# wildltr/ptranking

Hardware: AMD Instinct MI355X
Metric: queries/sec fwd+bwd LambdaRank, MSLR-WEB30K-shaped list_len=128 (higher is better)
Workload: dtype f32

## Files before the change

ptranking_amd/csrc/scorer_x6.hip:

```cpp
#include "ptr_mlp.h"

namespace ptr {

constexpr int kX6Pieces = kX6SliceBytes / 1024;
constexpr int kX6Ring = 6;

__host__ __device__ inline size_t x6_lds_bytes(int NL) { return (size_t)kX6Ring * kX6SliceBytes + ((size_t)NL * kHP + kHP + 16) * sizeof(float); }

__device__ __forceinline__ float relu1(float x) { return __builtin_amdgcn_fmed3f(x, 0.0f, 3.0e38f); }

__global__ void __launch_bounds__(256) x6_prep_kernel(const float *__restrict__ P, int F, int NL, uint8_t *__restrict__ img) {
    const int idx = blockIdx.x * 256 + threadIdx.x;
    const int n1 = x6_n1(F), ns = x6_nslices(F, NL);
    if (idx >= ns * kX6Rows * 4) return;
    const int g = idx & 3, row = (idx >> 2) % kX6Rows, sl = idx / (4 * kX6Rows);
    const int layer = sl < n1 ? 0 : 1 + (sl - n1) / 4, s = sl < n1 ? sl : (sl - n1) % 4;
    const int K = layer == 0 ? F : kH;
    const float *W = P + off_W(layer, F);
    Frag f[3];
#pragma unroll
    for (int h = 0; h < 2; ++h) {
        f32x4 v;
#pragma unroll
        for (int c = 0; c < 4; ++c) {
            const int k = layer == 0 ? 32 * s + 8 * g + 4 * h + c : 32 * s + 16 * h + 4 * g + c;
            v[c] = (row < kH && k < K) ? W[(size_t)row * K + k] : 0.0f;
            if (layer > 0 && row < kH && k == kH) v[c] = P[off_b(layer, F) + row];
        }
        split_pack4(v, f, 2 * h);
    }
#pragma unroll
    for (int p = 0; p < 3; ++p)
        *reinterpret_cast<u32x4 *>(img + (size_t)sl * kX6SliceBytes + (size_t)p * kX6PlaneBytes + (size_t)(row >> 4) * 1024 + g * 256 + (row & 15) * 16) = f[p].q;
}

using x6_rsrc = __amdgpu_buffer_rsrc_t;
__device__ __forceinline__ x6_rsrc x6_srd(void *p, uint32_t bytes) { return __builtin_amdgcn_make_buffer_rsrc(p, 0, (int)bytes, 0x00020000); }
__device__ __forceinline__ void x6_store16(x6_rsrc srd, uint32_t off, f32x4 v) {
    __builtin_amdgcn_raw_buffer_store_b128(__builtin_bit_cast(u32x4, v), srd, (int)off, 0, 0);
}
__device__ __forceinline__ f32x4 x6_load16(x6_rsrc srd, uint32_t voff, uint32_t soff) {
    return __builtin_bit_cast(f32x4, __builtin_amdgcn_raw_buffer_load_b128(srd, (int)voff, (int)soff, 0));
}
__device__ __forceinline__ void x6_store4(x6_rsrc srd, uint32_t off, float v) { __builtin_amdgcn_raw_buffer_store_b32(__builtin_bit_cast(uint32_t, v), srd, (int)off, 0, 0); }
constexpr uint32_t kX6Oob = 0xFFFFC000u;
constexpr uint64_t kX6BufLimit = 0xFFFFC000ull;

#define X6_MFMA(A, B, C) __builtin_amdgcn_mfma_f32_16x16x32_bf16((A).v, (B).v, (C), 0, 0, 0)

#define X6_SB() __builtin_amdgcn_sched_barrier(0)
#define X6_TSTRIDE 1024
#define X6_MIX(NM, NV)                                                                                     \
    do {                                                                                                   \
        _Pragma("unroll") for (int i_ = 0; i_ < (NM); ++i_) {                                              \
            __builtin_amdgcn_sched_group_barrier(0x008, 1, 0);                                             \
            __builtin_amdgcn_sched_group_barrier(0x002, (NV), 0);                                          \
        }                                                                                                  \
    } while (0)
template <int... Ks> struct X6K {};
template <int R, int K0, int... Ks> constexpr int x6_kget(X6K<K0, Ks...>) { if constexpr (R == 0) return K0; else return x6_kget<R - 1>(X6K<Ks...>{}); }

template <bool TRAIN, bool STORE, int DT>
__global__ void __launch_bounds__(16 / DT * 64, DT == 4 ? 1 : 2)
mlp_fwd_x6_kernel(const float *__restrict__ X, const float *__restrict__ P, const uint8_t *__restrict__ img, MlpArgs a,
                  float *__restrict__ preds, float *__restrict__ acts) {
    extern __shared__ __attribute__((aligned(16))) uint8_t smem_x6[];
    constexpr int NW = 16 / DT, RPT = 16 * DT, PW = (kX6Pieces + NW - 1) / NW;
    const int F = a.F, NL = a.NL, R = a.R;
    float *Bs = reinterpret_cast<float *>(smem_x6 + (size_t)kX6Ring * kX6SliceBytes);
    float *Wo = Bs + (size_t)NL * kHP;
    const int tid = threadIdx.x;
    for (int i = tid; i < NL * kHP; i += NW * 64) { const int l = i / kHP, c = i - l * kHP; Bs[i] = c < kH ? P[off_b(l, F) + c] : 0.0f; }
    for (int i = tid; i < kHP + 16; i += NW * 64) Wo[i] = i < kH ? P[off_wout(NL, F) + i] : (i == kHP ? P[off_wout(NL, F) + kH] : 0.0f);
    __syncthreads();
    const float b_out = Wo[kHP];

    const int lane = tid & 63, j = lane & 15, g = lane >> 4, wave = __builtin_amdgcn_readfirstlane(tid >> 6);
    const int ntiles = (R + RPT - 1) / RPT;
    const uint32_t thr = drop_thr(a.p_drop);
    const float scale = TRAIN ? 1.0f / (1.0f - a.p_drop) : 1.0f;
    const int n1 = x6_n1(F), ns = n1 + 4 * (NL - 1);
    const uint32_t ring = lds_byte_addr(smem_x6);
    const uint32_t lane_a = ring + (uint32_t)(lane * 16);

    int dma_slice = 0, dma_slot = 0;
    auto dma_issue = [&]() __attribute__((always_inline)) {
        const uint8_t *src = img + (size_t)dma_slice * kX6SliceBytes + lane * 16;
        const uint32_t dst = ring + (uint32_t)dma_slot * kX6SliceBytes;
#pragma unroll
        for (int i = 0; i < PW; ++i) {
            int q = wave * PW + i;
            q = q < kX6Pieces ? q : kX6Pieces - 1;
            glds16(src + q * 1024, __builtin_amdgcn_readfirstlane(dst + (uint32_t)q * 1024));
        }
        dma_slice = dma_slice + 1 == ns ? 0 : dma_slice + 1;
        dma_slot = dma_slot + 1 == kX6Ring ? 0 : dma_slot + 1;
    };
#pragma unroll 1
    for (int d = 0; d < kX6Ring - 1; ++d) dma_issue();
    static_assert(kX6Ring == 6 && (PW == 3 || PW == 6), "the vmcnt immediates below are PW * (kX6Ring - 2) and PW * (kX6Ring - 3) (+ the store margin)");
    if constexpr (STORE && DT == 2) {
#pragma unroll
        for (int i = 0; i < 6; ++i)
            glds16(img + (size_t)i * 1024 + lane * 16, __builtin_amdgcn_readfirstlane(ring + (uint32_t)(kX6Ring - 1) * kX6SliceBytes + (uint32_t)i * 1024));
    }
    if constexpr (DT == 4) asm volatile("s_waitcnt vmcnt(24)\n\ts_barrier" ::: "memory");
    else if constexpr (STORE) asm volatile("s_waitcnt vmcnt(18)\n\ts_barrier" ::: "memory");
    else asm volatile("s_waitcnt vmcnt(12)\n\ts_barrier" ::: "memory");
    int cur_slot = 0;
#ifdef PTR_X6_TRACE
    unsigned long long *trace = reinterpret_cast<unsigned long long *>(const_cast<uint8_t *>(img) + (size_t)ns * kX6SliceBytes) + wave * 256;
    int nstamp = 0;
#define X6_STAMP() do { if (blockIdx.x == 0 && lane == 0 && nstamp < 254) { trace[nstamp++] = clock64(); trace[nstamp & 1 ? 255 : 254] = wall_clock64(); if (nstamp == 1) trace[253] = wall_clock64(); } } while (0)
#else
#define X6_STAMP() do { } while (0)
#endif
    auto slice_sync = [&]() __attribute__((always_inline)) -> uint32_t {
        X6_STAMP();
        if constexpr (DT == 4) { if constexpr (STORE) asm volatile("s_waitcnt vmcnt(46)\n\ts_barrier" ::: "memory"); else asm volatile("s_waitcnt vmcnt(18)\n\ts_barrier" ::: "memory"); }
        else if constexpr (STORE) asm volatile("s_waitcnt vmcnt(23)\n\ts_barrier" ::: "memory");
        else asm volatile("s_waitcnt vmcnt(9)\n\ts_barrier" ::: "memory");
        X6_STAMP();
        dma_issue();
        cur_slot = cur_slot + 1 == kX6Ring ? 0 : cur_slot + 1;
        return lane_a + (uint32_t)cur_slot * kX6SliceBytes;
    };

    uint32_t bs_base = lds_byte_addr(Bs) + (uint32_t)g * 16;
    asm volatile("" : "+v"(bs_base));
    uint32_t wo_delta = (uint32_t)NL * (kHP * 4);
    asm volatile("" : "+s"(wo_delta));
    auto lds4 = [](uint32_t base, int byte_off) __attribute__((always_inline)) { return *reinterpret_cast<lds_f32x4 *>((uintptr_t)(base + (uint32_t)byte_off)); };
    const uint32_t nrt = (uint32_t)act_row_tiles(R), layer_bytes = nrt * (uint32_t)(kActTile * 4);
    const x6_rsrc xsrd = x6_srd(const_cast<float *>(X), (uint32_t)R * (uint32_t)(F * 4));
    const x6_rsrc psrd = x6_srd(preds, (uint32_t)R * 4u);
    const x6_rsrc asrd = x6_srd(acts, STORE ? (uint32_t)NL * layer_bytes : 0u);
    f32x4 acc[kMT][DT];
    Frag bp[4][DT][3];
    Frag bfx[2][DT][3];
    f32x4 raw[2][DT][2];
    Frag af[2][3];
    using I0 = std::integral_constant<int, 0>; using I1 = std::integral_constant<int, 1>;

    auto read_a = [&](Frag (&buf)[3], uint32_t abase, int mt) __attribute__((always_inline)) {
#pragma unroll
        for (int p = 0; p < 3; ++p) buf[p].q = *reinterpret_cast<lds_u32x4 *>((uintptr_t)(abase + (uint32_t)(p * kX6PlaneBytes + mt * 1024)));
    };
    auto mma_tile = [&](const Frag (&buf)[3], auto mt_, const Frag (&bf)[DT][3]) __attribute__((always_inline)) {
        constexpr int mt = decltype(mt_)::value;
#pragma unroll
        for (int q = 0; q < 6; ++q)
#pragma unroll
            for (int dt = 0; dt < DT; ++dt) acc[mt][dt] = X6_MFMA(buf[kSixA[q]], bf[dt][kSixB[q]], acc[mt][dt]);
    };
    auto mma_tile_tail = [&](const Frag (&buf)[3], auto mt_, const Frag (&bf)[DT][3]) __attribute__((always_inline)) {
        constexpr int mt = decltype(mt_)::value;
#pragma unroll
        for (int q = 0; q < 6; ++q)
#pragma unroll
            for (int dt = 0; dt < DT; ++dt)
                acc[mt][dt] = __builtin_amdgcn_mfma_f32_16x16x16bf16_1k(__builtin_bit_cast(i16x4, u32x2{buf[kSixA[q]].u[0], buf[kSixA[q]].u[1]}),
                                                                         __builtin_bit_cast(i16x4, u32x2{bf[dt][kSixB[q]].u[0], bf[dt][kSixB[q]].u[1]}), acc[mt][dt], 0, 0, 0);
    };
    auto slice_step = [&](auto ap_, uint32_t abase, const Frag (&bf)[DT][3], auto &&work, auto ks_, auto late_, auto tail_) __attribute__((always_inline)) -> uint32_t {
        constexpr int AP = decltype(ap_)::value;
        constexpr bool LATE = decltype(late_)::value;
        constexpr bool TAIL16 = decltype(tail_)::value;
        uint32_t nb = 0;
        static_for<kMT>([&](auto r_) __attribute__((always_inline)) {
            constexpr int r = decltype(r_)::value;
            constexpr int K = x6_kget<r>(decltype(ks_){});
            if constexpr (r == 3) nb = slice_sync();
            if constexpr (!LATE) {
                if constexpr (r < kMT - 1) read_a(af[AP ^ ((r + 1) & 1)], abase, r + 1);
                else read_a(af[AP ^ 1], nb, 0);
                X6_SB();
            }
            if constexpr (TAIL16) mma_tile_tail(af[AP ^ (r & 1)], r_, bf); else mma_tile(af[AP ^ (r & 1)], r_, bf);
            work(r_);
            if constexpr (K > 0) X6_MIX(6 * DT, K);
            X6_SB();
            if constexpr (LATE) {
                if constexpr (r < kMT - 1) read_a(af[AP ^ ((r + 1) & 1)], abase, r + 1);
                else read_a(af[AP ^ 1], nb, 0);
                X6_SB();
            }
        });
        return nb;
    };
    using Early = std::false_type;
    using Full = std::false_type;
    using Tail16 = std::true_type;
    using LateE = std::bool_constant<TRAIN>;
    using KNone = X6K<0, 0, 0, 0, 0, 0, 0>;
    auto nowork = [](auto) __attribute__((always_inline)) {};

    const int npass = (ntiles + NW * (int)gridDim.x - 1) / (NW * (int)gridDim.x);
    auto tile_of = [&](int it) __attribute__((always_inline)) { return (it * (int)gridDim.x + (int)blockIdx.x) * NW + wave; };
    uint32_t jX = (uint32_t)j * (uint32_t)(F * 4) + (uint32_t)g * 32, l16 = (uint32_t)(j * 64 + g * 16);
    uint32_t jH = (uint32_t)j * kDropRowMul + (uint32_t)g * kDropFgMul + a.seed_lo, jK = jH + (uint32_t)g * kDropFgMul;
    asm volatile("" : "+v"(jX), "+v"(l16), "+v"(jH), "+v"(jK));
    auto load_xq = [&](f32x4 (&rw)[DT][2], int t32, int s, int q) __attribute__((always_inline)) {
        const int dt = q >> 1, h = q & 1;
        const int left = F * 4 - 128 * s - 16 * h;
        const int ng = left <= 0 ? 0 : (left + 31) >> 5;
        const uint64_t cmask = ng >= 4 ? ~0ull : ((1ull << (16 * ng)) - 1ull);
        const uint64_t m = __builtin_amdgcn_ballot_w64(j < R - t32 - 16 * dt) & cmask;
        const uint32_t vo = __builtin_amdgcn_inverse_ballot_w64(m) ? jX : kX6Oob;
        const uint32_t so = (uint32_t)(t32 + 16 * dt) * (uint32_t)(F * 4);
        rw[dt][h] = x6_load16(xsrd, vo, so + (uint32_t)(128 * s + 16 * h));
    };
    auto make_bq = [&](const f32x4 (&rw)[DT][2], int t32, int s, Frag (&bf)[DT][3], int q) __attribute__((always_inline)) {
        const int dt = q >> 1, h = q & 1;
        f32x4 v = rw[dt][h];
        if constexpr (TRAIN) {
            uint32_t w0, w1;
            drop_bits_key(jK + ((uint32_t)(t32 + 16 * dt) * kDropRowMul + (uint32_t)(8 * s + h) * kDropFgMul), a.seed_hi, w0, w1);
            v = drop4(v, w0, w1, thr, scale);
        }
        split_pack4(v, bf[dt], 2 * h);
    };
    auto bias_init = [&]() __attribute__((always_inline)) {
#pragma unroll
        for (int mt = 0; mt < kMT; ++mt) {
            const f32x4 b4 = lds4(bs_base, 64 * mt);
            acc[mt][0] = b4; acc[mt][1] = b4;
        }
    };

    {
        const int t0 = tile_of(0) * RPT;
#pragma unroll
        for (int q = 0; q < 2 * DT; ++q) { load_xq(raw[0], t0, 0, q); load_xq(raw[1], t0, n1 > 1 ? 1 : 0, q); }
#pragma unroll
        for (int q = 0; q < 2 * DT; ++q) { make_bq(raw[0], t0, 0, bfx[0], q); load_xq(raw[0], t0, n1 > 2 ? 2 : 0, q); }
    }
    bias_init();
    uint32_t abase = lane_a;
    read_a(af[0], abase, 0);
    constexpr int KX = TRAIN ? 4 : 2, KE = TRAIN ? 9 : 5;

#pragma unroll 1
    for (int it = 0; it < npass; ++it) {
        const int tile = tile_of(it), tile_next = tile_of(it + 1);
        const int t32 = tile * RPT, t32n = tile_next * RPT;
        auto store_off = [&](int layer, int dt) __attribute__((always_inline)) {
            const uint32_t rt = (uint32_t)(t32 + 16 * dt) >> 4;
            uint32_t o = rt < nrt ? l16 + (rt * (uint32_t)(kActTile * 4) + (uint32_t)layer * layer_bytes) : kX6Oob;
            asm volatile("" : "+v"(o));
            return o;
        };
        auto epilogue = [&](auto mt_, int site) __attribute__((always_inline)) {
            constexpr int mt = decltype(mt_)::value;
#pragma unroll
            for (int dt = 0; dt < DT; ++dt) {
                f32x4 h = acc[mt][dt];
                acc[mt][dt] = f32x4{0.0f, 0.0f, 0.0f, 0.0f};
#pragma unroll
                for (int c = 0; c < 4; ++c) h[c] = relu1(h[c]);
                if constexpr (TRAIN) {
                    uint32_t w0, w1;
                    drop_bits_key(jH + ((uint32_t)(t32 + 16 * dt) * kDropRowMul + (uint32_t)(4 * mt) * kDropFgMul + (uint32_t)site * kDropSiteMul), a.seed_hi, w0, w1);
                    h = drop4(h, w0, w1, thr, scale);
                }
                if constexpr (STORE) {
                    f32x4 o = h;
                    if (mt == kMT - 1 && g == 1) o[0] = 1.0f;
                    x6_store16(asrd, store_off(site - 1, dt) + X6_TSTRIDE * mt, o);
                }
                split_pack4(h, bp[mt >> 1][dt], 2 * (mt & 1));
                if (mt == kMT - 1) {
                    bp[3][dt][0].u[0] |= g == 1 ? 0x3F80u : 0u;
                }
            }
        };
        float sc[DT];
#pragma unroll
        for (int dt = 0; dt < DT; ++dt) sc[dt] = 0.0f;
        auto epilogue_out = [&](auto mt_) __attribute__((always_inline)) {
            constexpr int mt = decltype(mt_)::value;
            const f32x4 w4 = lds4(bs_base + wo_delta, 64 * mt);
            const f32x4 bn = lds4(bs_base, 64 * mt);
#pragma unroll
            for (int dt = 0; dt < DT; ++dt) {
                f32x4 h = acc[mt][dt];
                acc[mt][dt] = bn;
#pragma unroll
                for (int c = 0; c < 4; ++c) { h[c] = relu1(h[c]); sc[dt] = fmaf(h[c], w4[c], sc[dt]); }
                if constexpr (STORE) x6_store16(asrd, store_off(NL - 1, dt) + X6_TSTRIDE * mt, h);
            }
        };

        auto l1_step = [&](auto par_, int s) __attribute__((always_inline)) {
            constexpr int PAR = decltype(par_)::value;
            abase = slice_step(par_, abase, bfx[PAR], [&](auto r_) __attribute__((always_inline)) {
                constexpr int r = decltype(r_)::value;
                auto quarter = [&](int q) __attribute__((always_inline)) { make_bq(raw[PAR ^ 1], t32, s + 1, bfx[PAR ^ 1], q); load_xq(raw[PAR ^ 1], t32, s + 3 < n1 ? s + 3 : 0, q); };
                if constexpr (DT == 2) {
                    constexpr int q = r == 0 ? 0 : r == 1 ? 1 : r == 3 ? 2 : r == 4 ? 3 : -1;
                    if constexpr (q >= 0) quarter(q);
                } else {
                    if constexpr (r == 0) { quarter(0); quarter(1); } else quarter(r + 1);
                }
            }, std::conditional_t<DT == 2, X6K<KX, KX, 0, KX, KX, 0, 0>, X6K<KX, KX / 2, KX / 2, KX / 2, KX / 2, KX / 2, KX / 2>>{}, Early{}, Full{});
        };
        auto l1_last = [&](auto par_) __attribute__((always_inline)) {
            constexpr int PAR = decltype(par_)::value;
            abase = slice_step(par_, abase, bfx[PAR], [&](auto r_) __attribute__((always_inline)) {
                constexpr int r = decltype(r_)::value;
                if constexpr (r > 0) epilogue(std::integral_constant<int, r - 1>{}, 1);
            }, X6K<0, KE, KE, KE, KE, KE, KE>{}, LateE{}, Full{});
            epilogue(std::integral_constant<int, kMT - 1>{}, 1);
            if constexpr (PAR == 0) {
#pragma unroll
                for (int p = 0; p < 3; ++p) af[0][p].q = af[1][p].q;
            }
        };
        int s = 0;
        for (; s + 2 <= n1 - 1; s += 2) { l1_step(I0{}, s); l1_step(I1{}, s + 1); }
        if (s < n1 - 1) { l1_step(I0{}, s); l1_last(I1{}); } else { l1_last(I0{}); }

        auto hidden = [&](auto lastlayer_, int l) __attribute__((always_inline)) {
            constexpr bool LAST = decltype(lastlayer_)::value;
            abase = slice_step(I0{}, abase, bp[0], nowork, KNone{}, Early{}, Full{});
            abase = slice_step(I1{}, abase, bp[1], nowork, KNone{}, Early{}, Full{});
            if constexpr (LAST) {
#pragma unroll
                for (int q = 0; q < 2 * DT; ++q) { load_xq(raw[0], t32n, 0, q); load_xq(raw[1], t32n, n1 > 1 ? 1 : 0, q); }
                X6_SB();
            }
            abase = slice_step(I0{}, abase, bp[2], nowork, KNone{}, Early{}, Full{});
            if constexpr (LAST) {
                abase = slice_step(I1{}, abase, bp[3], [&](auto r_) __attribute__((always_inline)) {
                    constexpr int r = decltype(r_)::value;
                    auto quarter = [&](int q) __attribute__((always_inline)) { make_bq(raw[0], t32n, 0, bfx[0], q); load_xq(raw[0], t32n, n1 > 2 ? 2 : 0, q); };
                    if constexpr (DT == 2) { if constexpr (r < 4) quarter(r); }
                    else if constexpr (r < 4) { quarter(2 * r); quarter(2 * r + 1); }
                    if constexpr (r > 0) epilogue_out(std::integral_constant<int, r - 1>{});
                }, X6K<KX, KX + 1, KX + 1, KX + 1, 1, 1, 1>{}, LateE{}, Tail16{});
                epilogue_out(std::integral_constant<int, kMT - 1>{});
            } else {
                abase = slice_step(I1{}, abase, bp[3], [&](auto r_) __attribute__((always_inline)) {
                    constexpr int r = decltype(r_)::value;
                    if constexpr (r > 0) epilogue(std::integral_constant<int, r - 1>{}, l + 1);
                }, X6K<0, KE, KE, KE, KE, KE, KE>{}, LateE{}, Tail16{});
                epilogue(std::integral_constant<int, kMT - 1>{}, l + 1);
            }
        };
#pragma unroll 1
        for (int l = 1; l < NL - 1; ++l) hidden(std::false_type{}, l);
        hidden(std::true_type{}, NL - 1);
#pragma unroll
        for (int dt = 0; dt < DT; ++dt) {
            float t = sc[dt];
            t += __shfl_xor(t, 16, 64);
            t += __shfl_xor(t, 32, 64);
            x6_store4(psrd, (g == 0 && j < R - t32 - 16 * dt) ? (uint32_t)(t32 + 16 * dt + j) * 4u : kX6Oob, t + b_out);
        }
    }
    asm volatile("s_waitcnt vmcnt(0)" ::: "memory");
}

bool x6_supported(int F, int NL) { return F % 4 == 0 && F >= 4 && NL >= 2 && NL <= kMaxLayers && x6_lds_bytes(NL) <= 160 * 1024; }

}

extern "C" size_t ptr_mlp_x6_ws_bytes(int F, int NL) {
    return ptr::x6_supported(F, NL) ? (size_t)ptr::x6_nslices(F, NL) * ptr::kX6SliceBytes + 16384 : 0;
}

extern "C" int ptr_mlp_forward_x6(const float *X, const float *params, int R, int F, int NL, int train, float p_drop, uint64_t seed,
                                  float *preds, float *acts, void *wimg, void *stream) {
    return ptr::mlp_forward_x6_impl(X, params, R, F, NL, train, p_drop, seed, preds, acts, wimg, true, stream);
}

int ptr::mlp_forward_x6_impl(const float *X, const float *params, int R, int F, int NL, int train, float p_drop, uint64_t seed, float *preds, float *acts,
                             void *wimg, bool prep, void *stream) {
    using namespace ptr;
    const char *who = "ptr_mlp_forward_x6";
    if (R < 0 || F <= 0 || NL < 1 || NL > kMaxLayers) { set_error("%s: bad shape R=%d F=%d NL=%d", who, R, F, NL); return PTR_ERR_INVALID_ARG; }
    if (!(p_drop >= 0.0f && p_drop < 1.0f)) { set_error("%s: dropout p=%g out of [0,1)", who, (double)p_drop); return PTR_ERR_INVALID_ARG; }
    if (!x6_supported(F, NL)) { set_error("%s: F=%d NL=%d is outside the bf16x6 scorer's range (F %% 4 == 0, 2 <= NL <= 8)", who, F, NL); return PTR_ERR_UNSUPPORTED; }
    if (R > 0 && (!X || !params || !preds || !wimg || (train && !acts))) { set_error("%s: NULL pointer", who); return PTR_ERR_INVALID_ARG; }
    if ((reinterpret_cast<uintptr_t>(X) & 15) || (reinterpret_cast<uintptr_t>(wimg) & 15) || (acts && (reinterpret_cast<uintptr_t>(acts) & 15))) {
        set_error("%s: X, acts and wimg must be 16-byte aligned", who); return PTR_ERR_INVALID_ARG;
    }
    if (R == 0) return 0;
    if ((uint64_t)R * (uint64_t)F * 4 >= kX6BufLimit) {
        set_error("%s: R * F * 4 bytes of X exceed the 4 GB a buffer resource addresses (R=%d, F=%d): split the batch", who, R, F);
        return PTR_ERR_UNSUPPORTED;
    }
    if (train && (uint64_t)NL * (uint64_t)act_layer_floats(R) * 4 >= kX6BufLimit) {
        set_error("%s: NL * ceil16(R) * 448 bytes of activations exceed the 4 GB a buffer resource addresses (R=%d): split the batch", who, R);
        return PTR_ERR_UNSUPPORTED;
    }
    MlpArgs a{R, F, NL, train ? p_drop : 0.0f, (uint32_t)seed, (uint32_t)(seed >> 32)};
    hipStream_t st = as_stream(stream);
    if (prep) {
        const int nthreads = x6_nslices(F, NL) * kX6Rows * 4;
        hipLaunchKernelGGL(x6_prep_kernel, dim3((nthreads + 255) / 256), dim3(256), 0, st, params, F, NL, reinterpret_cast<uint8_t *>(wimg));
        if (int e = check_hip(hipGetLastError(), who)) return e;
    }
    const size_t lds = x6_lds_bytes(NL);
    constexpr int dt = 2, nw = 16 / dt, rpt = 16 * dt;
    const int ntiles = (R + rpt - 1) / rpt, nblk = (ntiles + nw - 1) / nw;
    const int grid = nblk < num_cus() ? nblk : num_cus();
    auto launch = [&](auto kern) -> int {
        if (int e = allow_lds(kern, lds)) return e;
        hipLaunchKernelGGL(kern, dim3(grid), dim3(nw * 64), lds, st, X, params, reinterpret_cast<const uint8_t *>(wimg), a, preds, acts);
        return check_hip(hipGetLastError(), who);
    };
    return train ? launch(mlp_fwd_x6_kernel<true, true, 2>) : launch(mlp_fwd_x6_kernel<false, false, 2>);
}
```

Before: 5.444 million.

## Derive per-site exact vmcnt waits from a compile-time ledger of outstanding loads

Replaces the single conservative s_waitcnt vmcnt immediate used at every slice sync with per-site immediates. They are computed at compile time by a ledger that counts the outstanding global loads and stores issued by each pipeline step (layer-1 X loads, epilogue activation stores, last-layer X prefetch, output stores). Waits can now be looser where more unrelated ops are in flight, so the weight-ring DMA wait stalls less. It also drops the extra dummy prologue loads for STORE and restricts the kernel to DT==2. The risk is a wrong count in the ledger, which could either cause a race or leave the waits over-conservative.

```diff
diff --git a/ptranking_amd/csrc/ptr_x6_waits.h b/ptranking_amd/csrc/ptr_x6_waits.h
--- /dev/null
+++ b/ptranking_amd/csrc/ptr_x6_waits.h
@@ -0,0 +1,125 @@
+#pragma once
+
+namespace ptr {
+namespace x6w {
+
+constexpr int kRing = 6;
+constexpr int kAhead = kRing - 2;
+constexpr int kPW = 3;
+constexpr int kQuarters = 4;
+constexpr int kDocTiles = 2;
+constexpr int kRegions = 7;
+constexpr int kSyncRegion = 3;
+constexpr int kVmcntMax = 63;
+
+enum Step { L1, L1_LAST, HID, HID_EPI, HID_X, HID_OUT };
+constexpr int kFront = -1;
+constexpr int kBehind = kRegions;
+
+constexpr int ops(bool store, Step k, int r) {
+    switch (k) {
+    case L1:       return (r == 0 || r == 1 || r == 3 || r == 4) ? 1 : 0;
+    case L1_LAST:
+    case HID_EPI:  return store && r >= 1 ? kDocTiles : 0;
+    case HID:      return 0;
+    case HID_X:    return r == kFront ? 2 * kQuarters * 2 : 0;
+    case HID_OUT:  return (r >= 0 && r < kQuarters ? 1 : 0)
+                        + (store && r >= 1 ? kDocTiles : 0)
+                        + (r == kBehind ? kDocTiles : 0);
+    }
+    return 0;
+}
+struct Sums { int pre[6], post[6]; };
+constexpr Sums sums(bool store) {
+    Sums t{};
+    for (int k = 0; k < 6; ++k) {
+        for (int r = kFront; r < kSyncRegion; ++r) t.pre[k] += ops(store, (Step)k, r);
+        for (int r = kSyncRegion; r <= kBehind; ++r) t.post[k] += ops(store, (Step)k, r);
+    }
+    return t;
+}
+constexpr Sums kSums[2] = {sums(false), sums(true)};
+constexpr int pre(bool store, Step k) { return kSums[store].pre[k]; }
+constexpr int post(bool store, Step k) { return kSums[store].post[k]; }
+
+constexpr int nsteps(int n1, int NL) { return n1 + 4 * (NL - 1); }
+constexpr Step step_at(int n1, int NL, int i) {
+    if (i < n1) return i == n1 - 1 ? L1_LAST : L1;
+    const int layer = (i - n1) / 4, pos = (i - n1) % 4;
+    const bool last = layer == NL - 2;
+    return pos < 2 ? HID : pos == 2 ? (last ? HID_X : HID) : (last ? HID_OUT : HID_EPI);
+}
+constexpr int kPrologueLoads = 3 * kQuarters;
+constexpr int kPrologueWait = kAhead * kPW;
+
+constexpr int exact(bool store, int n1, int NL, bool first, int i) {
+    int n = pre(store, step_at(n1, NL, i));
+    for (int k = 1; k <= kAhead; ++k) {
+        int j = i - k, before = 0, behind = 0;
+        if (j < 0 && first) behind = j == -1 ? kPrologueLoads : 0;
+        else {
+            if (j < 0) j += nsteps(n1, NL);
+            before = pre(store, step_at(n1, NL, j));
+            behind = post(store, step_at(n1, NL, j));
+        }
+        n += k < kAhead ? before + kPW + behind : behind;
+    }
+    return n;
+}
+
+constexpr bool at_site(int n1, int NL, bool first, int i, bool layer1, bool epi, int pos, bool flag) {
+    if (layer1 != (i < n1)) return false;
+    if (layer1) return epi == (i == n1 - 1) && pos == (i < kAhead ? i : kAhead) && (pos == kAhead || flag == first);
+    const int layer = (i - n1) / 4;
+    return epi == (layer == NL - 2) && pos == (i - n1) % 4 && flag == (layer == 0 && n1 >= kAhead);
+}
+constexpr int kEnumN1 = 2 * kAhead, kEnumNL = 4;
+constexpr int site_fold(bool store, bool layer1, bool epi, int pos, bool flag, bool want_max) {
+    int m = -1;
+    for (int n1 = 1; n1 <= kEnumN1; ++n1)
+        for (int NL = 2; NL <= kEnumNL; ++NL)
+            for (int f = 0; f < 2; ++f)
+                for (int i = 0; i < nsteps(n1, NL); ++i) {
+                    if (!at_site(n1, NL, f != 0, i, layer1, epi, pos, flag)) continue;
+                    const int e = exact(store, n1, NL, f != 0, i);
+                    if (m < 0 || (want_max ? e > m : e < m)) m = e;
+                }
+    return m;
+}
+constexpr int site(bool store, bool layer1, bool epi, int pos, bool flag) { return site_fold(store, layer1, epi, pos, flag, false); }
+constexpr bool site_exact(bool store, bool layer1, bool epi, int pos, bool flag) {
+    return site_fold(store, layer1, epi, pos, flag, false) == site_fold(store, layer1, epi, pos, flag, true);
+}
+constexpr int used(bool store, int n1, int NL, bool first, int i) {
+    if (i < n1) return site(store, true, i == n1 - 1, i < kAhead ? i : kAhead, i < kAhead && first);
+    const int layer = (i - n1) / 4;
+    return site(store, false, layer == NL - 2, (i - n1) % 4, layer == 0 && n1 >= kAhead);
+}
+
+constexpr bool all_sites(bool store, bool check_exact) {
+    for (int epi = 0; epi < 2; ++epi)
+        for (int pos = 0; pos <= kAhead; ++pos)
+            for (int flag = 0; flag < 2; ++flag) {
+                const int w = site(store, true, epi != 0, pos, flag != 0);
+                if (w < 0 || w > kVmcntMax) return false;
+                if (check_exact && !site_exact(store, true, epi != 0, pos, flag != 0)) return false;
+                if (pos < 4) {
+                    const int h = site(store, false, epi != 0, pos, flag != 0);
+                    if (h < kAhead * kPW - kPW || h > kVmcntMax) return false;
+                    if (check_exact && flag && !site_exact(store, false, epi != 0, pos, true)) return false;
+                }
+            }
+    return true;
+}
+static_assert(all_sites(true, false), "training: an immediate does not fit vmcnt's 6 bits, or a site is unreachable");
+static_assert(all_sites(false, false), "evaluation: an immediate does not fit vmcnt's 6 bits, or a site is unreachable");
+static_assert(all_sites(true, true), "training: a layer-1 site (or a hidden site behind a long layer 1) sees more than one history");
+static_assert(all_sites(false, true), "evaluation: a layer-1 site (or a hidden site behind a long layer 1) sees more than one history");
+static_assert(exact(true, 5, 3, false, 0) == 47 && exact(true, 5, 3, false, 2) == 39 && exact(true, 5, 3, false, 8) == 23
+              && exact(true, 5, 3, false, 11) == 39 && exact(true, 5, 3, false, 12) == 42, "training ledger");
+static_assert(exact(false, 5, 3, false, 0) == 33 && exact(false, 5, 3, false, 5) == 19 && exact(false, 5, 3, false, 8) == 9
+              && exact(false, 5, 3, false, 11) == 25 && exact(false, 5, 3, false, 12) == 28, "evaluation ledger");
+static_assert(site(true, false, false, 0, false) == kRegions * kDocTiles + (kAhead - 1) * kPW && site(false, false, false, 0, false) == (kAhead - 1) * kPW, "");
+
+}
+}
diff --git a/ptranking_amd/csrc/scorer_x6.hip b/ptranking_amd/csrc/scorer_x6.hip
--- a/ptranking_amd/csrc/scorer_x6.hip
+++ b/ptranking_amd/csrc/scorer_x6.hip
@@ -1,4 +1,5 @@
 #include "ptr_mlp.h"
+#include "ptr_x6_waits.h"
 
 namespace ptr {
 
@@ -8,6 +9,11 @@
 __host__ __device__ inline size_t x6_lds_bytes(int NL) { return (size_t)kX6Ring * kX6SliceBytes + ((size_t)NL * kHP + kHP + 16) * sizeof(float); }
 
 __device__ __forceinline__ float relu1(float x) { return __builtin_amdgcn_fmed3f(x, 0.0f, 3.0e38f); }
+
+template <int N> __device__ __forceinline__ void x6_vm_wait() {
+    static_assert(N >= 0 && N <= x6w::kVmcntMax, "vmcnt has 6 bits on gfx9");
+    asm volatile("s_waitcnt vmcnt(%0)" ::"n"(N) : "memory");
+}
 
 __global__ void __launch_bounds__(256) x6_prep_kernel(const float *__restrict__ P, int F, int NL, uint8_t *__restrict__ img) {
     const int idx = blockIdx.x * 256 + threadIdx.x;
@@ -98,15 +104,9 @@
     };
 #pragma unroll 1
     for (int d = 0; d < kX6Ring - 1; ++d) dma_issue();
-    static_assert(kX6Ring == 6 && (PW == 3 || PW == 6), "the vmcnt immediates below are PW * (kX6Ring - 2) and PW * (kX6Ring - 3) (+ the store margin)");
-    if constexpr (STORE && DT == 2) {
-#pragma unroll
-        for (int i = 0; i < 6; ++i)
-            glds16(img + (size_t)i * 1024 + lane * 16, __builtin_amdgcn_readfirstlane(ring + (uint32_t)(kX6Ring - 1) * kX6SliceBytes + (uint32_t)i * 1024));
-    }
-    if constexpr (DT == 4) asm volatile("s_waitcnt vmcnt(24)\n\ts_barrier" ::: "memory");
-    else if constexpr (STORE) asm volatile("s_waitcnt vmcnt(18)\n\ts_barrier" ::: "memory");
-    else asm volatile("s_waitcnt vmcnt(12)\n\ts_barrier" ::: "memory");
+    static_assert(DT == 2 && kX6Ring == x6w::kRing && PW == x6w::kPW && kMT == x6w::kRegions, "the vmcnt ledger (ptr_x6_waits.h) counts this schedule");
+    x6_vm_wait<x6w::kPrologueWait>();
+    asm volatile("s_barrier" ::: "memory");
     int cur_slot = 0;
 #ifdef PTR_X6_TRACE
     unsigned long long *trace = reinterpret_cast<unsigned long long *>(const_cast<uint8_t *>(img) + (size_t)ns * kX6SliceBytes) + wave * 256;
@@ -115,11 +115,10 @@
 #else
 #define X6_STAMP() do { } while (0)
 #endif
-    auto slice_sync = [&]() __attribute__((always_inline)) -> uint32_t {
+    auto slice_sync = [&](auto &&wait) __attribute__((always_inline)) -> uint32_t {
         X6_STAMP();
-        if constexpr (DT == 4) { if constexpr (STORE) asm volatile("s_waitcnt vmcnt(46)\n\ts_barrier" ::: "memory"); else asm volatile("s_waitcnt vmcnt(18)\n\ts_barrier" ::: "memory"); }
-        else if constexpr (STORE) asm volatile("s_waitcnt vmcnt(23)\n\ts_barrier" ::: "memory");
-        else asm volatile("s_waitcnt vmcnt(9)\n\ts_barrier" ::: "memory");
+        wait();
+        asm volatile("s_barrier" ::: "memory");
         X6_STAMP();
         dma_issue();
         cur_slot = cur_slot + 1 == kX6Ring ? 0 : cur_slot + 1;
@@ -162,7 +161,7 @@
                 acc[mt][dt] = __builtin_amdgcn_mfma_f32_16x16x16bf16_1k(__builtin_bit_cast(i16x4, u32x2{buf[kSixA[q]].u[0], buf[kSixA[q]].u[1]}),
                                                                          __builtin_bit_cast(i16x4, u32x2{bf[dt][kSixB[q]].u[0], bf[dt][kSixB[q]].u[1]}), acc[mt][dt], 0, 0, 0);
     };
-    auto slice_step = [&](auto ap_, uint32_t abase, const Frag (&bf)[DT][3], auto &&work, auto ks_, auto late_, auto tail_) __attribute__((always_inline)) -> uint32_t {
+    auto slice_step = [&](auto ap_, uint32_t abase, const Frag (&bf)[DT][3], auto &&work, auto ks_, auto late_, auto tail_, auto &&wait) __attribute__((always_inline)) -> uint32_t {
         constexpr int AP = decltype(ap_)::value;
         constexpr bool LATE = decltype(late_)::value;
         constexpr bool TAIL16 = decltype(tail_)::value;
@@ -170,7 +169,7 @@
         static_for<kMT>([&](auto r_) __attribute__((always_inline)) {
             constexpr int r = decltype(r_)::value;
             constexpr int K = x6_kget<r>(decltype(ks_){});
-            if constexpr (r == 3) nb = slice_sync();
+            if constexpr (r == x6w::kSyncRegion) nb = slice_sync(wait);
             if constexpr (!LATE) {
                 if constexpr (r < kMT - 1) read_a(af[AP ^ ((r + 1) & 1)], abase, r + 1);
                 else read_a(af[AP ^ 1], nb, 0);
@@ -291,6 +290,14 @@
             }
         };
 
+        auto l1_wait = [&](auto epi_, int s) __attribute__((always_inline)) {
+            constexpr bool EPI = decltype(epi_)::value;
+            if (s >= x6w::kAhead) x6_vm_wait<x6w::site(STORE, true, EPI, x6w::kAhead, false)>();
+            else static_for<x6w::kAhead>([&](auto k_) __attribute__((always_inline)) {
+                constexpr int k = decltype(k_)::value;
+                if (s == k) { if (it == 0) x6_vm_wait<x6w::site(STORE, true, EPI, k, true)>(); else x6_vm_wait<x6w::site(STORE, true, EPI, k, false)>(); }
+            });
+        };
         auto l1_step = [&](auto par_, int s) __attribute__((always_inline)) {
             constexpr int PAR = decltype(par_)::value;
             abase = slice_step(par_, abase, bfx[PAR], [&](auto r_) __attribute__((always_inline)) {
@@ -302,14 +309,15 @@
                 } else {
                     if constexpr (r == 0) { quarter(0); quarter(1); } else quarter(r + 1);
                 }
-            }, std::conditional_t<DT == 2, X6K<KX, KX, 0, KX, KX, 0, 0>, X6K<KX, KX / 2, KX / 2, KX / 2, KX / 2, KX / 2, KX / 2>>{}, Early{}, Full{});
+            }, std::conditional_t<DT == 2, X6K<KX, KX, 0, KX, KX, 0, 0>, X6K<KX, KX / 2, KX / 2, KX / 2, KX / 2, KX / 2, KX / 2>>{}, Early{}, Full{},
+               [&]() __attribute__((always_inline)) { l1_wait(std::false_type{}, s); });
         };
         auto l1_last = [&](auto par_) __attribute__((always_inline)) {
             constexpr int PAR = decltype(par_)::value;
             abase = slice_step(par_, abase, bfx[PAR], [&](auto r_) __attribute__((always_inline)) {
                 constexpr int r = decltype(r_)::value;
                 if constexpr (r > 0) epilogue(std::integral_constant<int, r - 1>{}, 1);
-            }, X6K<0, KE, KE, KE, KE, KE, KE>{}, LateE{}, Full{});
+            }, X6K<0, KE, KE, KE, KE, KE, KE>{}, LateE{}, Full{}, [&]() __attribute__((always_inline)) { l1_wait(std::true_type{}, n1 - 1); });
             epilogue(std::integral_constant<int, kMT - 1>{}, 1);
             if constexpr (PAR == 0) {
 #pragma unroll
@@ -322,14 +330,19 @@
 
         auto hidden = [&](auto lastlayer_, int l) __attribute__((always_inline)) {
             constexpr bool LAST = decltype(lastlayer_)::value;
-            abase = slice_step(I0{}, abase, bp[0], nowork, KNone{}, Early{}, Full{});
-            abase = slice_step(I1{}, abase, bp[1], nowork, KNone{}, Early{}, Full{});
+            auto hid_wait = [&](auto pos_) __attribute__((always_inline)) {
+                constexpr int pos = decltype(pos_)::value;
+                if (l == 1 && n1 >= x6w::kAhead) x6_vm_wait<x6w::site(STORE, false, LAST, pos, true)>(); else x6_vm_wait<x6w::site(STORE, false, LAST, pos, false)>();
+            };
+            using I2 = std::integral_constant<int, 2>; using I3 = std::integral_constant<int, 3>;
+            abase = slice_step(I0{}, abase, bp[0], nowork, KNone{}, Early{}, Full{}, [&]() __attribute__((always_inline)) { hid_wait(I0{}); });
+            abase = slice_step(I1{}, abase, bp[1], nowork, KNone{}, Early{}, Full{}, [&]() __attribute__((always_inline)) { hid_wait(I1{}); });
             if constexpr (LAST) {
 #pragma unroll
                 for (int q = 0; q < 2 * DT; ++q) { load_xq(raw[0], t32n, 0, q); load_xq(raw[1], t32n, n1 > 1 ? 1 : 0, q); }
                 X6_SB();
             }
-            abase = slice_step(I0{}, abase, bp[2], nowork, KNone{}, Early{}, Full{});
+            abase = slice_step(I0{}, abase, bp[2], nowork, KNone{}, Early{}, Full{}, [&]() __attribute__((always_inline)) { hid_wait(I2{}); });
             if constexpr (LAST) {
                 abase = slice_step(I1{}, abase, bp[3], [&](auto r_) __attribute__((always_inline)) {
                     constexpr int r = decltype(r_)::value;
@@ -337,13 +350,13 @@
                     if constexpr (DT == 2) { if constexpr (r < 4) quarter(r); }
                     else if constexpr (r < 4) { quarter(2 * r); quarter(2 * r + 1); }
                     if constexpr (r > 0) epilogue_out(std::integral_constant<int, r - 1>{});
-                }, X6K<KX, KX + 1, KX + 1, KX + 1, 1, 1, 1>{}, LateE{}, Tail16{});
+                }, X6K<KX, KX + 1, KX + 1, KX + 1, 1, 1, 1>{}, LateE{}, Tail16{}, [&]() __attribute__((always_inline)) { hid_wait(I3{}); });
                 epilogue_out(std::integral_constant<int, kMT - 1>{});
             } else {
                 abase = slice_step(I1{}, abase, bp[3], [&](auto r_) __attribute__((always_inline)) {
                     constexpr int r = decltype(r_)::value;
                     if constexpr (r > 0) epilogue(std::integral_constant<int, r - 1>{}, l + 1);
-                }, X6K<0, KE, KE, KE, KE, KE, KE>{}, LateE{}, Tail16{});
+                }, X6K<0, KE, KE, KE, KE, KE, KE>{}, LateE{}, Tail16{}, [&]() __attribute__((always_inline)) { hid_wait(I3{}); });
                 epilogue(std::integral_constant<int, kMT - 1>{}, l + 1);
             }
         };
```

Result: no change. 5.413 million (-0.6%).
